# szaguldo-kamaz/FRI-ReinforcementLearning-C

Measured on AMD Instinct MI355X. Metric: rule-distance evals/sec (rules x envs), higher is better.
Workload: dtype f64; 1 GPU; cfg4_acrobot_64k_x_8k_per_gpu; nant=5, universe_len=41, rules_per_env=65536, envs_per_gpu=8192, exact_hits=4, dist_backend=none, world_size=1

## Files before the change

### fri-reinforcementlearning-c_amd/csrc/episode_kernel.h

```cpp
#pragma once

#include <type_traits>

#include "envs.h"
#include "sweeps.h"

namespace frirl {

struct NoIo {};
struct ExtIo : frirl_hip_agent_io {
    const int32_t *teacher;
};
template <bool EXT>
using IoArg = std::conditional_t<EXT, ExtIo, NoIo>;

__device__ __forceinline__ int taught_action(const ExtIo &io, int e, int A, int chosen)
{
    if (!io.teacher) return chosen;
    const int32_t k = io.teacher[e];
    return (k >= 0 && k < A) ? k : chosen;
}

struct StepShared {
    double q_ant[FRIRL_HIP_MAX_NANT];
// ... 10 lines not shown
};

__device__ __forceinline__ bool frirl_no_spread_candidates(const frirl_hip_agent &ag) { return (ag.debug_flags & 1) != 0; }

template <int NANT, int BLOCK, bool TRACK = false, class COLS, class POW>
__device__ int update_sarsa_block(const COLS &cols, const double *__restrict__ u, const double *__restrict__ ve, int U, double *__restrict__ base,
                                  int maxR, int32_t *nrules_e, const frirl_hip_agent &ag, StepShared &sh, double reward,
                                  bool qp_known, double qp, int32_t *fus_e, double *rant_e, BlockRed<BLOCK> &red,
                                  const QResult *rn_known, uint16_t *uidx_e, POW p, SpreadCand *slot, double *spread_ant_e = nullptr, int32_t *spread_R_e = nullptr)
{
    const int R = *nrules_e;
    double q1[NANT], q2[NANT];
#pragma unroll
    for (int k = 0; k < NANT; k++) { q1[k] = sh.ve1[k]; q2[k] = sh.ve2[k]; }
    double *qcol = base + (size_t)NANT * maxR;

    if (!qp_known) {
        const QResult rp = sweep_q<NANT, BLOCK>(cols, qcol, R, q2, p, red);
        qp = (rp.hit != FRIRL_HIP_NO_HIT) ? qcol[rp.hit] : rp.vagc / rp.ws;
    }
    const QResult rn = rn_known ? *rn_known : sweep_q<NANT, BLOCK, TRACK>(cols, qcol, R, q1, p, red, ag.weight_significant, slot);
    const double qnow = (rn.hit != FRIRL_HIP_NO_HIT) ? qcol[rn.hit] : rn.vagc / rn.ws;
    const double qdiff = ag.alpha * (reward + ag.gamma * qp - qnow);
    int fus = *fus_e;
    __syncthreads();

    if (qdiff > ag.qdiff_pos_boundary || qdiff < ag.qdiff_neg_boundary) {
        if (threadIdx.x < NANT) {
            const int k = threadIdx.x;
            const double r = check_possible_states(sh.q_ant[k], ag.grid_values + (size_t)k * FRIRL_HIP_MAX_GRID, ag.grid_len[k]);
            sh.rant[k] = r;
            const double *uni = u + (size_t)k * U;
            const unsigned j = snap_index(uni, U, r, universe_div(uni, U));
            sh.idx3[k] = j;
            sh.ve3[k] = ve[(size_t)k * U + j];
        }
        __syncthreads();
        double q3[NANT];
        bool same = true;
#pragma unroll
        for (int k = 0; k < NANT; k++) { q3[k] = sh.ve3[k]; same = same && (q3[k] == q1[k]); }
        QResult rr = rn;
        if (!same) rr = sweep_q<NANT, BLOCK>(cols, qcol, R, q3, p, red);
        if (rr.hit == FRIRL_HIP_NO_HIT) {
            if (R >= maxR) return FRIRL_HIP_UPD_FULL;
            const double rconc = rr.vagc / rr.ws;
            if (threadIdx.x < NANT) {
                base[(size_t)threadIdx.x * maxR + R] = q3[threadIdx.x];
                if (uidx_e) uidx_e[(size_t)threadIdx.x * maxR + R] = (uint16_t)sh.idx3[threadIdx.x];
                if (rant_e) rant_e[(size_t)threadIdx.x * maxR + R] = sh.rant[threadIdx.x];
            }
            if (threadIdx.x == 0) {
                qcol[R] = rconc + qdiff;
                *nrules_e = R + 1;
                *fus_e = 1;
            }
            return FRIRL_HIP_UPD_INSERTED;
        }
        fus = 0;
    }

    int rules = R;
    if (fus) rules--;
    int status;
    if (rn.hit != FRIRL_HIP_NO_HIT && (ag.skip_rules == 0 || (ag.skip_rules == 1 && (int)rn.hit < rules))) {
        if (threadIdx.x == 0) qcol[rn.hit] = qnow + qdiff;
        status = FRIRL_HIP_UPD_EXACT;
    } else if (ag.skip_rules == 1 && rn.hit != FRIRL_HIP_NO_HIT && (int)rn.hit == rules) {
        status = FRIRL_HIP_UPD_SKIPPED;
    } else {
        if (ag.skip_rules == 0) fus = 0;
        const int r_skip = fus ? R - 1 : -1;
        if (rn.hit == FRIRL_HIP_NO_HIT) {
            if (spread_ant_e && threadIdx.x < NANT) spread_ant_e[threadIdx.x] = sh.q_ant[threadIdx.x];
            if (spread_R_e && threadIdx.x == 0) *spread_R_e = R;
        }
        const bool from_cand = TRACK && rn.tracked && rn.hit == FRIRL_HIP_NO_HIT && !frirl_no_spread_candidates(ag) &&
                               spread_from_candidates<BLOCK>(slot[threadIdx.x], qcol, rn.ws, qnow, qdiff, ag.weight_significant, r_skip, red);
        if (!from_cand) sweep_update<NANT, BLOCK>(cols, qcol, R, q1, p, rn.ws, qnow, qdiff, ag.weight_significant, r_skip);
        status = FRIRL_HIP_UPD_SPREAD;
    }
    if (threadIdx.x == 0) *fus_e = fus;
    return status;
}

template <int NANT, int AMAX, int BLOCK, bool IDX, bool PN, bool EXT = false>
__global__ __launch_bounds__(BLOCK) void episode_begin_kernel(const double *__restrict__ u, const double *__restrict__ ve, int U,
                                                               const double *__restrict__ rb, const uint16_t *__restrict__ uidx,
                                                               const int32_t *__restrict__ nrules,
                                                               int maxR, const frirl_hip_agent ag, const frirl_hip_envs ev, const IoArg<EXT> io)
{
    constexpr int NS = NANT - 1;
    const int e = blockIdx.x;
    if constexpr (EXT) {
        if (io.reset && !io.reset[e]) return;
    }
    extern __shared__ double tab_s[];
    __shared__ double q_s[NS];
    __shared__ GbaScratch<AMAX, BLOCK> gs;
    if (IDX) for (int i = threadIdx.x; i < NANT * U; i += BLOCK) tab_s[i] = ve[i];
    if (threadIdx.x < NS) {
        double v;
        if constexpr (EXT) v = io.obs[(size_t)e * NS + threadIdx.x];
        else v = ev.start_states ? ev.start_states[(size_t)e * NS + threadIdx.x] : ag.values_def[threadIdx.x];
        ev.states[(size_t)e * NS + threadIdx.x] = v;
        ev.q_ant[(size_t)e * NANT + threadIdx.x] = v;
        q_s[threadIdx.x] = observe_ve(u, ve, U, threadIdx.x, v);
    }
    if ((int)threadIdx.x < ag.A) gs.ave[threadIdx.x] = ag.action_ve[threadIdx.x];
    __syncthreads();
    double q[NS];
#pragma unroll
    for (int k = 0; k < NS; k++) q[k] = q_s[k];
    const double *base = rb + (size_t)e * (NANT + 1) * maxR;
    const double *qcol = base + (size_t)NANT * maxR;
    const auto cols = ColsSel<IDX>::make(base, uidx + (IDX ? (size_t)e * NANT * maxR : 0), tab_s, maxR, U);
    const auto pw = PowSel<PN, NANT>::make(ag.p > 0 ? ag.p : NANT);
    int a0;
    if constexpr (AMAX == 24) {
        __shared__ BlockRed<BLOCK> red;
        double dummy[NANT] = {};
        a0 = sweep_gba_many<NANT, AMAX, BLOCK, false>(cols, qcol, nrules[e], q, dummy, pw, ag.A, gs, red, nullptr);
    } else if constexpr (AMAX > 8) {
        __shared__ BlockRed<BLOCK> red;
        double dummy[NANT] = {};
        a0 = sweep_gba_wide<NANT, 8, AMAX, BLOCK, false>(cols, qcol, nrules[e], q, dummy, pw, ag.A, gs, red, nullptr);
    } else {
        a0 = sweep_gba<NANT, AMAX, BLOCK>(cols, qcol, nrules[e], q, pw, ag.A, gs);
    }
    if (threadIdx.x == 0) {
        const uint32_t epi = ev.episode ? (uint32_t)(ev.episode[e] + 1) : 0u;
        if (ev.episode) ev.episode[e] = (int32_t)epi;
        a0 = e_greedy(ag, a0, (uint32_t)e, epi, 0u);
        if constexpr (EXT) a0 = taught_action(io, e, ag.A, a0);
        ev.q_ant[(size_t)e * NANT + NS] = ag.grid_values[(size_t)NS * FRIRL_HIP_MAX_GRID + a0];
        if constexpr (EXT) {
            io.action_out[e] = ag.grid_values[(size_t)NS * FRIRL_HIP_MAX_GRID + a0];
            if (io.action_idx) io.action_idx[e] = a0;
        }
        ev.done[e] = 0;
        ev.ep_steps[e] = 0;
        ev.ep_reward[e] = 0.0;
        if (ev.status) ev.status[e] = FRIRL_HIP_UPD_INACTIVE;
    }
}

#ifndef FRIRL_STEP_WAVES_N3
#define FRIRL_STEP_WAVES_N3 6
#endif
#ifndef FRIRL_STEP_SAME_CELL
#define FRIRL_STEP_SAME_CELL 1
#endif
constexpr int step_min_waves(int nant, int amax) { return (nant <= 3 && amax <= 4) ? FRIRL_STEP_WAVES_N3 : (amax > 8 ? 3 : 4); }

#ifdef FRIRL_STEP_TIMING
static __device__ long long g_step_timing[4 * 65536];
#endif

template <int NANT, int AMAX, int BLOCK, bool IDX, bool PN, bool TRACK, bool EXT = false>
__global__ __launch_bounds__(BLOCK, step_min_waves(NANT, AMAX)) void episode_step_kernel(const double *__restrict__ u, const double *__restrict__ ve, int U,
                                                              double *__restrict__ rb, uint16_t *__restrict__ uidx, int32_t *__restrict__ nrules,
                                                              int maxR, const frirl_hip_agent ag, const frirl_hip_envs ev, const IoArg<EXT> io)
{
    constexpr int NS = NANT - 1;
    const int e = blockIdx.x;
#ifdef FRIRL_STEP_TIMING
    static_assert(!EXT, "step timing: demo kernels only");
    const long long tm0 = wall_clock64();
#endif
    if (ev.done[e]) {
        if (threadIdx.x == 0 && ev.status) ev.status[e] = FRIRL_HIP_UPD_INACTIVE;
        return;
    }
    extern __shared__ double tab_s[];
    __shared__ StepShared sh;
    __shared__ BlockRed<BLOCK> red;
    __shared__ GbaScratch<AMAX, BLOCK> gs;
    __shared__ SpreadCand cand_s[TRACK ? BLOCK : 1];
    if (IDX) for (int i = threadIdx.x; i < NANT * U; i += BLOCK) tab_s[i] = ve[i];
    if (threadIdx.x == 0) {
        double s[FRIRL_HIP_MAX_NANT], q[FRIRL_HIP_MAX_NANT];
        if constexpr (EXT) {
            (void)s;
            for (int i = 0; i < NANT; i++) sh.q_ant[i] = ev.q_ant[(size_t)e * NANT + i];
            for (int i = 0; i < NS; i++) sh.cur_states[i] = io.obs[(size_t)e * NS + i];
            sh.reward = io.reward[e];
            sh.success = io.success[e];
            if (io.q_obs) for (int i = 0; i < NS; i++) q[i] = io.q_obs[(size_t)e * NS + i];
            else env_quantize(FRIRL_HIP_ENV_EXTERNAL, NS, ag.grid_values, ag.grid_len, ag.grid_div, sh.cur_states, q);
        } else {
            for (int i = 0; i < NS; i++) s[i] = ev.states[(size_t)e * NS + i];
            for (int i = 0; i < NANT; i++) sh.q_ant[i] = ev.q_ant[(size_t)e * NANT + i];
            env_do_action(ag.env_kind, sh.q_ant[NS], s, sh.cur_states);
            env_get_reward(ag.env_kind, sh.cur_states, sh.reward, sh.success);
            env_quantize(ag.env_kind, NS, ag.grid_values, ag.grid_len, ag.grid_div, sh.cur_states, q);
        }
        for (int i = 0; i < NS; i++) sh.cur_q_ant[i] = q[i];
    }
    if ((int)threadIdx.x < ag.A) gs.ave[threadIdx.x] = ag.action_ve[threadIdx.x];
    __syncthreads();
    if (threadIdx.x < NANT) sh.ve1[threadIdx.x] = observe_ve(u, ve, U, threadIdx.x, sh.q_ant[threadIdx.x]);
    if (threadIdx.x < NS) sh.ve2[threadIdx.x] = observe_ve(u, ve, U, threadIdx.x, sh.cur_q_ant[threadIdx.x]);
    __syncthreads();
    double q[NS];
#pragma unroll
    for (int k = 0; k < NS; k++) q[k] = sh.ve2[k];
    double *base = rb + (size_t)e * (NANT + 1) * maxR;
    const double *qcol = base + (size_t)NANT * maxR;
    uint16_t *uidx_e = uidx ? uidx + (size_t)e * NANT * maxR : nullptr;
    const auto cols = ColsSel<IDX>::make(base, uidx_e, tab_s, maxR, U);
    double q1[NANT];
#pragma unroll
    for (int k = 0; k < NANT; k++) q1[k] = sh.ve1[k];
    const auto pw = PowSel<PN, NANT>::make(ag.p > 0 ? ag.p : NANT);
    QResult rn;
    int ap;
    if constexpr (AMAX == 24) ap = sweep_gba_many<NANT, AMAX, BLOCK, true>(cols, qcol, nrules[e], q, q1, pw, ag.A, gs, red, &rn);
    else if constexpr (AMAX > 8) ap = sweep_gba_wide<NANT, 8, AMAX, BLOCK, true, TRACK>(cols, qcol, nrules[e], q, q1, pw, ag.A, gs, red, &rn, ag.weight_significant, cand_s);
    else {
        bool same_cell = NS > 0 && FRIRL_STEP_SAME_CELL != 0;
#pragma unroll
        for (int k = 0; k < NS; k++) same_cell = same_cell && (q[k] == q1[k]);
        int apend = -1;
        for (int a = ag.A - 1; a >= 0; a--) if (gs.ave[a] == q1[NS]) apend = a;
        if (same_cell && apend >= 0) ap = sweep_gba_q<NANT, AMAX, BLOCK, TRACK, true>(cols, qcol, nrules[e], q, q1, pw, ag.A, gs, red, rn, ag.weight_significant, cand_s, apend);
        else ap = sweep_gba_q<NANT, AMAX, BLOCK, TRACK, false>(cols, qcol, nrules[e], q, q1, pw, ag.A, gs, red, rn, ag.weight_significant, cand_s);
    }
#ifdef FRIRL_STEP_TIMING
    const long long tm1 = wall_clock64();
#endif
    if (threadIdx.x == 0) {
        int chosen = e_greedy(ag, ap, (uint32_t)e, ev.episode ? (uint32_t)ev.episode[e] : 0u, (uint32_t)ev.ep_steps[e] + 1u);
        if constexpr (EXT) chosen = taught_action(io, e, ag.A, chosen);
        gs.best = chosen;
        sh.cur_q_ant[NS] = ag.grid_values[(size_t)NS * FRIRL_HIP_MAX_GRID + chosen];
        sh.ve2[NS] = gs.ave[chosen];
        if constexpr (EXT) {
            io.action_out[e] = sh.cur_q_ant[NS];
            if (io.action_idx) io.action_idx[e] = chosen;
        }
    }
    __syncthreads();
    const double qp = gs.actconc[gs.best];
    double *rant_e = ev.rant ? ev.rant + (size_t)e * NANT * maxR : nullptr;
    int st = FRIRL_HIP_UPD_INACTIVE;
    if (!ag.evaluate)
        st = update_sarsa_block<NANT, BLOCK, TRACK>(cols, u, ve, U, base, maxR, nrules + e, ag, sh, sh.reward, true, qp, ev.fus + e, rant_e, red, &rn, uidx_e, pw, cand_s,
                                                    ev.spread_ant ? ev.spread_ant + (size_t)e * NANT : nullptr, ev.spread_R ? ev.spread_R + e : nullptr);
    if (threadIdx.x < NS) ev.states[(size_t)e * NS + threadIdx.x] = sh.cur_states[threadIdx.x];
    if (threadIdx.x < NANT) ev.q_ant[(size_t)e * NANT + threadIdx.x] = sh.cur_q_ant[threadIdx.x];
    if (threadIdx.x == 0) {
        const int steps = ev.ep_steps[e] + 1;
        ev.ep_steps[e] = steps;
        ev.ep_reward[e] = ev.ep_reward[e] + sh.reward;
        if (sh.success == 1 || steps >= ag.max_steps) ev.done[e] = 1;
        if (ev.status) ev.status[e] = st;
#ifdef FRIRL_STEP_TIMING
        if (e < 65536) { g_step_timing[4 * e] = tm0; g_step_timing[4 * e + 1] = tm1; g_step_timing[4 * e + 2] = wall_clock64(); g_step_timing[4 * e + 3] = st; }
#endif
    }
}

template <int N, int AMAX, int BLOCK, bool BEGIN, bool EXT>
static void launch_episode_v(const frirl_hip_tables *t, const frirl_hip_rulebases *b, const frirl_hip_agent *ag, const frirl_hip_envs *ev,
                             hipStream_t s, const IoArg<EXT> &io)
{
    const bool idx = frirl::use_uidx(t, b) && (BLOCK >= 256 || sizeof(double) * t->nant * (size_t)t->U <= 4096);
    const size_t tab = idx ? sizeof(double) * t->nant * (size_t)t->U : 0;
    const bool pn = ag->p <= 0 || ag->p == N;
    constexpr bool CAN_TRACK = (N >= 4 && AMAX <= 4);
    const int st_opt = frirl_host::opts().step_track;
    const bool track = CAN_TRACK && (st_opt == 1 || (st_opt < 0 && b->maxR > 16384 + 512));
#define EP_GO(KERNEL, DYN, ...)                                                                                                                  \
    hipLaunchKernelGGL((frirl::KERNEL<N, AMAX, BLOCK, __VA_ARGS__, EXT>), dim3(b->E), dim3(BLOCK), DYN, s, t->u, t->ve, t->U, b->rb, b->uidx, b->nrules, \
                       b->maxR, *ag, *ev, io)
    if constexpr (BEGIN) {
        if (idx) { if (pn) EP_GO(episode_begin_kernel, tab, true, true); else EP_GO(episode_begin_kernel, tab, true, false); }
        else { if (pn) EP_GO(episode_begin_kernel, 0, false, true); else EP_GO(episode_begin_kernel, 0, false, false); }
    } else {
        if constexpr (CAN_TRACK) {
            if (track) {
                if (idx) { if (pn) EP_GO(episode_step_kernel, tab, true, true, true); else EP_GO(episode_step_kernel, tab, true, false, true); }
                else { if (pn) EP_GO(episode_step_kernel, 0, false, true, true); else EP_GO(episode_step_kernel, 0, false, false, true); }
                return;
            }
        }
        if (idx) { if (pn) EP_GO(episode_step_kernel, tab, true, true, false); else EP_GO(episode_step_kernel, tab, true, false, false); }
        else { if (pn) EP_GO(episode_step_kernel, 0, false, true, false); else EP_GO(episode_step_kernel, 0, false, false, false); }
    }
#undef EP_GO
}

template <int N, bool BEGIN, bool EXT = false>
static void launch_episode(const frirl_hip_tables *t, const frirl_hip_rulebases *b, const frirl_hip_agent *ag, const frirl_hip_envs *ev,
                           hipStream_t s, const IoArg<EXT> &io = IoArg<EXT>{})
{
    bool small = b->maxR <= 2048 || (b->maxR <= 16384 && b->E >= 4096);
    const int sw = frirl_host::opts().step_wave;
    if (sw >= 0) small = sw == 1;
    if (ag->A <= 4) { if (small) launch_episode_v<N, 4, 64, BEGIN, EXT>(t, b, ag, ev, s, io); else launch_episode_v<N, 4, 256, BEGIN, EXT>(t, b, ag, ev, s, io); }
    else if (ag->A <= 8) { if (small) launch_episode_v<N, 8, 64, BEGIN, EXT>(t, b, ag, ev, s, io); else launch_episode_v<N, 8, 256, BEGIN, EXT>(t, b, ag, ev, s, io); }
    else if (ag->A <= 24 && !frirl_host::opts().no_many) launch_episode_v<N, 24, 256, BEGIN, EXT>(t, b, ag, ev, s, io);
    else launch_episode_v<N, 32, 256, BEGIN, EXT>(t, b, ag, ev, s, io);
}

}
```

### fri-reinforcementlearning-c_amd/csrc/sweeps.h

```cpp
#pragma once

#include <stdlib.h>

#include <type_traits>

#include "device_common.h"

namespace frirl {

__device__ __forceinline__ double pow_int(double b, int p)
{
    double r = b;
    for (int i = 1; i < p; i++) r = r * b;
    return r;
}

template <bool UNROLLED_POWERS = false>
__device__ __forceinline__ double inv_dist_pow(double s, int p)
{
    double y = __builtin_amdgcn_rsq(s);
    const double t = s * y;
    const double e = __fma_rn(-t, y, 1.0);
    const double c = __fma_rn(0.375, e, 0.5);
    const double ce = c * e;
// ... 128 lines not shown
    using raw_t = double2;
    __device__ __forceinline__ raw_t raw(int k, int r) const { return pair(k, r); }
    __device__ __forceinline__ raw_t raw_shared(int k, int r) const { return load_col2_shared(base + (size_t)k * maxR + r); }
    __device__ __forceinline__ double2 decode(int, const raw_t &w) const { return w; }
};

#ifndef FRIRL_BUF_LOADS
#define FRIRL_BUF_LOADS 1
#endif
static constexpr int BUFFER_RSRC_DWORD3 = 0x00020000;
__device__ __forceinline__ __amdgpu_buffer_rsrc_t raw_buffer(const void *p)
{
    return __builtin_amdgcn_make_buffer_rsrc(const_cast<void *>(p), (short)0, (int)0x7fffffff, BUFFER_RSRC_DWORD3);
}
struct QColBuf {
    __amdgpu_buffer_rsrc_t rs;
    __device__ __forceinline__ explicit QColBuf(const double *qcol) : rs(raw_buffer(qcol)) {}
    __device__ __forceinline__ double2 load2(int r) const
    {
        const auto w = __builtin_amdgcn_raw_buffer_load_b128(rs, 8 * r, 0, 2);
        double2 v;
        v.x = __longlong_as_double((long long)(((unsigned long long)w[1] << 32) | w[0]));
        v.y = __longlong_as_double((long long)(((unsigned long long)w[3] << 32) | w[2]));
        return v;
    }
};

template <int HALF>
__device__ __forceinline__ double lds_table_entry(const double *tab_k, uint32_t w)
{
#if FRIRL_DECODE_MAD
    const uint32_t base = (uint32_t)(uintptr_t)(lds_cdouble *)tab_k;
    uint32_t a;
    if constexpr (HALF == 0) asm("v_mad_u32_u16 %0, %1, 8, %2 op_sel:[0,0,0,0]" : "=v"(a) : "v"(w), "s"(base));
    else asm("v_mad_u32_u16 %0, %1, 8, %2 op_sel:[1,0,0,0]" : "=v"(a) : "v"(w), "s"(base));
    return *(lds_cdouble *)(uintptr_t)a;
#else
    return tab_k[HALF ? (w >> 16) : (w & 0xFFFFu)];
#endif
}

struct ColsIdx {
    static constexpr bool GLOBAL_Q = true;
    const uint16_t *idx;
    const double *tab;
    int maxR, U;
    __device__ __forceinline__ double2 pair(int k, int r) const
    {
        const uint32_t w = __builtin_nontemporal_load(reinterpret_cast<const uint32_t *>(idx + (size_t)k * maxR + r));
        return lds_table_pair(tab + k * U, w);
    }
    using raw_t = uint32_t;
    __device__ __forceinline__ raw_t raw(int k, int r) const
    {
#if FRIRL_BUF_LOADS
        return __builtin_amdgcn_raw_buffer_load_b32(raw_buffer(idx), 2 * r, 2 * k * maxR, 2);
#else
        return __builtin_nontemporal_load(reinterpret_cast<const uint32_t *>(idx + (size_t)k * maxR + r));
#endif
    }
    __device__ __forceinline__ raw_t raw_shared(int k, int r) const { return *reinterpret_cast<const uint32_t *>(idx + (size_t)k * maxR + r); }
    __device__ __forceinline__ double2 decode(int k, raw_t w) const { return lds_table_pair(tab + k * U, w); }
};

struct ColsLds {
    static constexpr bool GLOBAL_Q = false;
    const double *base;
    int cap;
    __device__ __forceinline__ double2 pair(int k, int r) const { return *reinterpret_cast<const double2 *>(base + (size_t)k * cap + r); }
    using raw_t = double2;
    __device__ __forceinline__ raw_t raw(int k, int r) const { return pair(k, r); }
    __device__ __forceinline__ raw_t raw_shared(int k, int r) const { return pair(k, r); }
    __device__ __forceinline__ double2 decode(int, const raw_t &w) const { return w; }
};

template <bool IDX>
struct ColsSel;
template <>
struct ColsSel<false> {
    using type = ColsF64;
    static __device__ __forceinline__ type make(const double *base, const uint16_t *, const double *, int maxR, int) { return ColsF64{base, maxR}; }
};
template <>
struct ColsSel<true> {
    using type = ColsIdx;
    static __device__ __forceinline__ type make(const double *, const uint16_t *idx, const double *tab, int maxR, int U) { return ColsIdx{idx, tab, maxR, U}; }
};

static inline bool use_uidx(const frirl_hip_tables *t, const frirl_hip_rulebases *b)
{
    return b->uidx && t->U <= 65536 && sizeof(double) * t->nant * (size_t)t->U <= 48 * 1024 && b->maxR > 2048 && !frirl_host::opts().no_uidx;
}

template <int NDIM, class COLS>
__device__ __forceinline__ void sq_dist2(const COLS &cols, int r, const double (&q)[NDIM], double &a0, double &a1)
{
    double2 v[NDIM];
#pragma unroll
    for (int k = 0; k < NDIM; k++) v[k] = cols.pair(k, r);
    double d0 = q[0] - v[0].x, d1 = q[0] - v[0].y;
    a0 = d0 * d0;
    a1 = d1 * d1;
#pragma unroll
    for (int k = 1; k < NDIM; k++) {
        d0 = q[k] - v[k].x;
        d1 = q[k] - v[k].y;
        a0 = __fma_rn(d0, d0, a0);
        a1 = __fma_rn(d1, d1, a1);
    }
}

static constexpr double SPREAD_PREFILTER_SLACK = 1.0 - 1.0 / 1048576.0;

struct SpreadCand {
    double w1, w2, w3;
    unsigned r1, r2;
    __device__ __forceinline__ void clear() { w1 = w2 = w3 = 0.0; r1 = r2 = FRIRL_HIP_NO_HIT; }
    __device__ __forceinline__ void offer(double wi, unsigned r)
    {
        if (wi > w1) { w3 = w2; w2 = w1; r2 = r1; w1 = wi; r1 = r; }
        else if (wi > w2) { w3 = w2; w2 = wi; r2 = r; }
        else if (wi > w3) w3 = wi;
    }
};

__device__ __forceinline__ double wave_uniform(double v)
{
    const unsigned long long b = (unsigned long long)__double_as_longlong(v);
    const unsigned lo = (unsigned)__builtin_amdgcn_readfirstlane((int)(unsigned)b), hi = (unsigned)__builtin_amdgcn_readfirstlane((int)(unsigned)(b >> 32));
    return __longlong_as_double((long long)(((unsigned long long)hi << 32) | lo));
}

__device__ __forceinline__ void spread_track(SpreadCand *slots, double &T, double thr, double w0, double w1, unsigned r, double run)
{
    const bool p0 = w0 > T, p1 = w1 > T;
    if (__builtin_amdgcn_ballot_w64(p0 || p1) != 0ull) {
        SpreadCand *slot = slots + threadIdx.x;
        if (p0) slot->offer(w0, r);
        if (p1) slot->offer(w1, r + 1u);
        T = wave_uniform(thr * wave_sum_f64(run));
    }
}

__device__ __forceinline__ int wave_uniform_limit(int R) { return ((R + 2 * FRIRL_WAVE - 1) / (2 * FRIRL_WAVE)) * (2 * FRIRL_WAVE); }

struct QResult {
    unsigned hit;
    double vagc;
    double ws;
    bool tracked;
};

static constexpr double NO_RULE_STATE_PART = 1.0e300;
template <class POW>
__device__ __forceinline__ void q_pair(double a0, double a1, const double2 &c, unsigned r, POW pk, unsigned &best, double &sv, double &sw, double &tw0,
                                       double &tw1)
{
    if (__builtin_amdgcn_ballot_w64(a0 == 0.0 || a1 == 0.0) != 0ull) {
        if (a0 == 0.0) best = min(best, r);
        if (a1 == 0.0) best = min(best, r + 1u);
    }
    const double w0 = shepard_w(a0, pk), w1 = shepard_w(a1, pk);
    sv = __fma_rn(w0, c.x, sv);
    sw = sw + w0;
    sv = __fma_rn(w1, c.y, sv);
    sw = sw + w1;
    tw0 = w0;
    tw1 = w1;
}

template <int NANT, int BLOCK, bool TRACK = false, class COLS, class POW>
__device__ QResult sweep_q(const COLS &cols, const double *__restrict__ qcol, int R, const double (&q)[NANT], POW p, BlockRed<BLOCK> &red, double track_thr = 0.0,
                           SpreadCand *slot = nullptr)
{
    unsigned best = FRIRL_HIP_NO_HIT;
    double sv = 0.0, sw = 0.0;
    QResult res;
    res.tracked = TRACK;
    if (TRACK) slot[threadIdx.x].clear();
    track_thr = wave_uniform(track_thr * SPREAD_PREFILTER_SLACK);
    double T = 0.0;
    const auto pk = pin_pow(p);
    const int r_lim = TRACK ? wave_uniform_limit(R) : R;
    for (int r = 2 * (int)threadIdx.x; r < r_lim; r += 2 * BLOCK) {
        double tw0 = 0.0, tw1 = 0.0;
        if (!TRACK || r < R) {
            double a0, a1;
            sq_dist2<NANT>(cols, r, q, a0, a1);
            double2 c = load_col2(qcol + r);
            if (r + 1 >= R) { a1 = NO_RULE_STATE_PART; c.y = 0.0; }
            q_pair(a0, a1, c, (unsigned)r, pk, best, sv, sw, tw0, tw1);
        }
        if (TRACK) spread_track(slot, T, track_thr, tw0, tw1, (unsigned)r, sw);
    }
    res.hit = blk_min<BLOCK>(best, red);
    res.vagc = blk_sum<BLOCK>(sv, red);
    res.ws = blk_sum<BLOCK>(sw, red);
    return res;
}

template <int NANT, int BLOCK, class COLS, class POW>
__device__ void sweep_weights(const COLS &cols, int R, const double (&q)[NANT], POW p, double ws, double *__restrict__ weights)
{
    const double iws = 1.0 / ws;
    for (int r = 2 * (int)threadIdx.x; r < R; r += 2 * BLOCK) {
        double a0, a1;
        sq_dist2<NANT>(cols, r, q, a0, a1);
        const double w0 = shepard_w(a0, p) * iws;
        const double w1 = shepard_w(a1, p) * iws;
        if (r + 1 < R) {
            double2 w; w.x = w0; w.y = w1;
            *reinterpret_cast<double2 *>(weights + r) = w;
        } else weights[r] = w0;
    }
}

template <int NANT, int BLOCK, class COLS, class POW>
__device__ void sweep_update(const COLS &cols, double *__restrict__ qcol, int R, const double (&q)[NANT], POW p, double ws, double qnow,
                             double qdiff, double threshold, int r_skip)
{
    const double iws = 1.0 / ws;
    for (int r = 2 * (int)threadIdx.x; r < R; r += 2 * BLOCK) {
        double a0, a1;
        sq_dist2<NANT>(cols, r, q, a0, a1);
        const double w0 = shepard_w(a0, p) * iws;
        const double w1 = shepard_w(a1, p) * iws;
        if (w0 > threshold && r != r_skip) { const double t = qdiff * w0; qcol[r] = qnow + t; }
        if (r + 1 < R && w1 > threshold && r + 1 != r_skip) { const double t = qdiff * w1; qcol[r + 1] = qnow + t; }
    }
}

template <int BLOCK>
__device__ bool spread_from_candidates(const SpreadCand &cd, double *__restrict__ qcol, double ws, double qnow, double qdiff, double threshold, int r_skip,
                                       BlockRed<BLOCK> &red)
{
    const double iws = 1.0 / ws;
    const unsigned ovf = (cd.w3 * iws > threshold) ? 0u : 1u;
    if (blk_min<BLOCK>(ovf, red) == 0u) return false;
    if (cd.r1 != FRIRL_HIP_NO_HIT) {
        const double w = cd.w1 * iws;
        if (w > threshold && (int)cd.r1 != r_skip) { const double t = qdiff * w; qcol[cd.r1] = qnow + t; }
    }
    if (cd.r2 != FRIRL_HIP_NO_HIT) {
        const double w = cd.w2 * iws;
        if (w > threshold && (int)cd.r2 != r_skip) { const double t = qdiff * w; qcol[cd.r2] = qnow + t; }
    }
    return true;
}

template <int AMAX, int BLOCK>
struct GbaScratch {
    static constexpr int WAVES = BLOCK / FRIRL_WAVE;
    double v[WAVES][AMAX];
    double w[WAVES][AMAX];
    unsigned hit[AMAX];
    double actconc[AMAX];
    double ave[AMAX];
    double tv[AMAX], tw[AMAX];
    int best;
};

#ifndef FRIRL_GBA_FASTPATH
#define FRIRL_GBA_FASTPATH 1
#endif
template <class POW>
__device__ __forceinline__ void concl_pair_nohit(double av, const double2 &va, double s0, double s1, const double2 &c, POW p, double &sv, double &sw)
{
    const double e0 = av - va.x, e1 = av - va.y;
    const double d0 = __fma_rn(e0, e0, s0), d1 = __fma_rn(e1, e1, s1);
    const double w0 = shepard_w(d0, p), w1 = shepard_w(d1, p);
    sv = __fma_rn(w0, c.x, sv);
    sw = sw + w0;
    sv = __fma_rn(w1, c.y, sv);
    sw = sw + w1;
}
template <class POW>
__device__ __forceinline__ void concl_pair_nohit(double av, const double2 &va, double s0, double s1, const double2 &c, POW p, double &sv, double &sw, double &w0,
                                                 double &w1)
{
    const double e0 = av - va.x, e1 = av - va.y;
    const double d0 = __fma_rn(e0, e0, s0), d1 = __fma_rn(e1, e1, s1);
    w0 = shepard_w(d0, p); w1 = shepard_w(d1, p);
    sv = __fma_rn(w0, c.x, sv);
    sw = sw + w0;
    sv = __fma_rn(w1, c.y, sv);
    sw = sw + w1;
}
__device__ __forceinline__ bool wave_no_state_hit(bool second, double s0, double s1)
{
    return FRIRL_GBA_FASTPATH && __builtin_amdgcn_ballot_w64(!second || s0 == 0.0 || s1 == 0.0) == 0ull;
}

#ifndef FRIRL_STEP_PREFETCH
#define FRIRL_STEP_PREFETCH 1
#endif
static constexpr int STEP_PREFETCH = FRIRL_STEP_PREFETCH;
__device__ __forceinline__ void note_state_hits(unsigned *hit_s, const double *ave_s, int A, double s0, double s1, const double2 &va, unsigned r)
{
    if (__builtin_amdgcn_ballot_w64(s0 == 0.0 || s1 == 0.0) != 0ull) {
        for (int a = 0; a < A; a++) {
            const double ava = ave_s[a];
            if (s0 == 0.0 && ava == va.x) atomicMin(&hit_s[a], r);
            if (s1 == 0.0 && ava == va.y) atomicMin(&hit_s[a], r + 1u);
        }
    }
}

template <int NANT, int AMAX, int BLOCK, class COLS, class POW>
__device__ int sweep_gba(const COLS &cols, const double *__restrict__ qcol, int R, const double (&qs)[NANT - 1 > 0 ? NANT - 1 : 1], POW p, int A,
                         GbaScratch<AMAX, BLOCK> &s)
{
    constexpr int NS = NANT - 1;
    double sv[AMAX], sw[AMAX], av[AMAX];
#pragma unroll
    for (int a = 0; a < AMAX; a++) { sv[a] = 0.0; sw[a] = 0.0; av[a] = wave_uniform(s.ave[a < A ? a : 0]); }
    if ((int)threadIdx.x < AMAX) s.hit[threadIdx.x] = FRIRL_HIP_NO_HIT;
    __syncthreads();
    const auto pk = pin_pow(p);
    for (int r = 2 * (int)threadIdx.x; r < R; r += 2 * BLOCK) {
        double s0 = 0.0, s1 = 0.0;
        if (NS > 0) sq_dist2<(NS > 0 ? NS : 1)>(cols, r, qs, s0, s1);
        double2 va = cols.pair(NS, r);
        double2 c = load_col2(qcol + r);
        const bool second = (r + 1 < R);
        if (!second) { s1 = NO_RULE_STATE_PART; va.y = 0.0; c.y = 0.0; }
        note_state_hits(s.hit, s.ave, A, s0, s1, va, (unsigned)r);
#pragma unroll
        for (int a = 0; a < AMAX; a++)
            if (a < A) concl_pair_nohit(av[a], va, s0, s1, c, pk, sv[a], sw[a]);
    }
    const int lane = threadIdx.x & (FRIRL_WAVE - 1), wave = threadIdx.x / FRIRL_WAVE;
    wave_sum_f64_n(sv);
    wave_sum_f64_n(sw);
#pragma unroll
    for (int a = 0; a < AMAX; a++)
        if (a < A && lane == 0) { s.v[wave][a] = sv[a]; s.w[wave][a] = sw[a]; }
    __syncthreads();
    if ((int)threadIdx.x < A) {
        const int a = threadIdx.x;
        double tv = s.v[0][a], tw = s.w[0][a];
        for (int w = 1; w < GbaScratch<AMAX, BLOCK>::WAVES; w++) { tv = tv + s.v[w][a]; tw = tw + s.w[w][a]; }
        const unsigned th = s.hit[a];
        s.actconc[a] = (th != FRIRL_HIP_NO_HIT) ? qcol[th] : tv / tw;
    }
    __syncthreads();
    if (threadIdx.x == 0) {
        int best = 0;
        for (int a = 1; a < A; a++) if (s.actconc[best] < s.actconc[a]) best = a;
        s.best = best;
    }
    __syncthreads();
    return s.best;
}

template <int NANT, int AMAX, int BLOCK, bool TRACK = false, bool SAMES = false, class COLS, class POW>
__device__ int sweep_gba_q(const COLS &cols, const double *__restrict__ qcol, int R, const double (&qs_in)[NANT - 1 > 0 ? NANT - 1 : 1],
                           const double (&q1_in)[NANT], POW p, int A, GbaScratch<AMAX, BLOCK> &s, BlockRed<BLOCK> &red, QResult &qres, double track_thr = 0.0,
                           SpreadCand *slot = nullptr, int apend = 0)
{
    constexpr int NS = NANT - 1;
    double qs[NS > 0 ? NS : 1], q1[NANT];
#pragma unroll
    for (int k = 0; k < (NS > 0 ? NS : 1); k++) qs[k] = wave_uniform(qs_in[k]);
#pragma unroll
    for (int k = 0; k < NANT; k++) q1[k] = wave_uniform(q1_in[k]);
    if (TRACK) slot[threadIdx.x].clear();
    qres.tracked = TRACK;
    track_thr = wave_uniform(track_thr * SPREAD_PREFILTER_SLACK);
    double sv[AMAX], sw[AMAX], av[AMAX];
#pragma unroll
    for (int a = 0; a < AMAX; a++) { sv[a] = 0.0; sw[a] = 0.0; av[a] = wave_uniform(s.ave[a < A ? a : 0]); }
    if ((int)threadIdx.x < AMAX) s.hit[threadIdx.x] = FRIRL_HIP_NO_HIT;
    __syncthreads();
    const auto pk = pin_pow(p);
    unsigned qbest = FRIRL_HIP_NO_HIT;
    double qv = 0.0, qw = 0.0;
    constexpr int PD = STEP_PREFETCH;
    const QColBuf qb(qcol);
    auto ldq = [&](int r) {
        if constexpr (COLS::GLOBAL_Q && FRIRL_BUF_LOADS) return qb.load2(r);
        else return load_col2(qcol + r);
    };
    typename COLS::raw_t nraw[PD][NANT];
    double2 nc[PD];
#pragma unroll
    for (int u = 0; u < PD; u++) {
        const int r0 = 2 * (int)threadIdx.x + u * 2 * BLOCK;
        nc[u] = double2{0.0, 0.0};
        if (r0 < R) {
#pragma unroll
            for (int k = 0; k < NANT; k++) nraw[u][k] = cols.raw(k, r0);
            nc[u] = ldq(r0);
        }
    }
    double T = 0.0;
    const int r_lim = TRACK ? wave_uniform_limit(R) : R;
    auto rule_pair = [&](const int r, typename COLS::raw_t (&sraw)[NANT], double2 &sc) {
        const bool live = !TRACK || r < R;
        const bool second = (r + 1 < R);
        double2 v[NANT];
        double2 c = {0.0, 0.0};
        double tw0 = 0.0, tw1 = 0.0;
        if (live) {
            c = sc;
#pragma unroll
            for (int k = 0; k < NANT; k++) v[k] = cols.decode(k, sraw[k]);
            if (r + PD * 2 * BLOCK < R) {
#pragma unroll
                for (int k = 0; k < NANT; k++) sraw[k] = cols.raw(k, r + PD * 2 * BLOCK);
                sc = ldq(r + PD * 2 * BLOCK);
            }
            if constexpr (!SAMES) {
                double d0 = q1[0] - v[0].x, d1 = q1[0] - v[0].y;
                double a0 = d0 * d0, a1 = d1 * d1;
#pragma unroll
                for (int k = 1; k < NANT; k++) {
                    d0 = q1[k] - v[k].x; d1 = q1[k] - v[k].y;
                    a0 = __fma_rn(d0, d0, a0); a1 = __fma_rn(d1, d1, a1);
                }
                if (!second) { a1 = NO_RULE_STATE_PART; c.y = 0.0; }
                q_pair(a0, a1, c, (unsigned)r, pk, qbest, qv, qw, tw0, tw1);
            }
        }
        if constexpr (!SAMES) { if (TRACK) spread_track(slot, T, track_thr, tw0, tw1, (unsigned)r, qw); }
        if (live) {
            double s0, s1;
            {
                double d0 = qs[0] - v[0].x, d1 = qs[0] - v[0].y;
                s0 = d0 * d0; s1 = d1 * d1;
#pragma unroll
                for (int k = 1; k < NS; k++) {
                    d0 = qs[k] - v[k].x; d1 = qs[k] - v[k].y;
                    s0 = __fma_rn(d0, d0, s0); s1 = __fma_rn(d1, d1, s1);
                }
            }
            double2 va = v[NS];
            if (!second) { s1 = NO_RULE_STATE_PART; va.y = 0.0; c.y = 0.0; }
            note_state_hits(s.hit, s.ave, A, s0, s1, va, (unsigned)r);
#pragma unroll
            for (int a = 0; a < AMAX; a++)
                if (a < A) {
                    if constexpr (SAMES && TRACK) {
                        double w0, w1;
                        concl_pair_nohit(av[a], va, s0, s1, c, pk, sv[a], sw[a], w0, w1);
                        if (a == apend) { tw0 = w0; tw1 = w1; qw = sw[a]; }
                    } else {
                        concl_pair_nohit(av[a], va, s0, s1, c, pk, sv[a], sw[a]);
                    }
                }
        }
        if constexpr (SAMES) { if (TRACK) spread_track(slot, T, track_thr, tw0, tw1, (unsigned)r, qw); }
    };
    for (int r = 2 * (int)threadIdx.x; r < r_lim; r += PD * 2 * BLOCK) {
#pragma unroll
        for (int u = 0; u < PD; u++) {
            const int ru = r + u * 2 * BLOCK;
            if (ru < r_lim) rule_pair(ru, nraw[u], nc[u]);
        }
    }
    if constexpr (!SAMES) {
        qres.hit = blk_min<BLOCK>(qbest, red);
        qres.vagc = blk_sum<BLOCK>(qv, red);
        qres.ws = blk_sum<BLOCK>(qw, red);
    }
    const int lane = threadIdx.x & (FRIRL_WAVE - 1), wave = threadIdx.x / FRIRL_WAVE;
    wave_sum_f64_n(sv);
    wave_sum_f64_n(sw);
#pragma unroll
    for (int a = 0; a < AMAX; a++)
        if (a < A && lane == 0) { s.v[wave][a] = sv[a]; s.w[wave][a] = sw[a]; }
    __syncthreads();
    if ((int)threadIdx.x < A) {
        const int a = threadIdx.x;
        double tv = s.v[0][a], tw = s.w[0][a];
        for (int w = 1; w < GbaScratch<AMAX, BLOCK>::WAVES; w++) { tv = tv + s.v[w][a]; tw = tw + s.w[w][a]; }
        const unsigned th = s.hit[a];
        s.actconc[a] = (th != FRIRL_HIP_NO_HIT) ? qcol[th] : tv / tw;
        s.tv[a] = tv; s.tw[a] = tw;
    }
    __syncthreads();
    if constexpr (SAMES) { qres.hit = s.hit[apend]; qres.vagc = s.tv[apend]; qres.ws = s.tw[apend]; }
    if (threadIdx.x == 0) {
        int best = 0;
        for (int a = 1; a < A; a++) if (s.actconc[best] < s.actconc[a]) best = a;
        s.best = best;
    }
    __syncthreads();
    return s.best;
}

template <int NANT, int AMAX, int BLOCK, bool WITH_Q, class COLS, class POW>
__device__ int sweep_gba_many(const COLS &cols, const double *__restrict__ qcol, int R, const double (&qs)[NANT - 1 > 0 ? NANT - 1 : 1],
                              const double (&q1)[NANT], POW p, int A, GbaScratch<AMAX, BLOCK> &s, BlockRed<BLOCK> &red, QResult *qres)
{
    constexpr int NS = NANT - 1;
    constexpr int G = 3;
    static_assert(AMAX % G == 0 && AMAX % 12 == 0, "groups of three actions, reduction passes of twelve");
    const int lane = threadIdx.x & (FRIRL_WAVE - 1), wave = __builtin_amdgcn_readfirstlane((int)(threadIdx.x / FRIRL_WAVE));
    double sv[AMAX], sw[AMAX], av[AMAX];
#pragma unroll
    for (int a = 0; a < AMAX; a++) { sv[a] = 0.0; sw[a] = 0.0; av[a] = wave_uniform(s.ave[a < A ? a : A - 1]); }
    if ((int)threadIdx.x < AMAX) s.hit[threadIdx.x] = FRIRL_HIP_NO_HIT;
    __syncthreads();
    unsigned qbest = FRIRL_HIP_NO_HIT;
    double qv = 0.0, qw = 0.0;
    const auto pk = pin_pow(p);
    const QColBuf qb(qcol);
    auto ldq = [&](int r) {
        if constexpr (COLS::GLOBAL_Q && FRIRL_BUF_LOADS) return qb.load2(r);
        else return load_col2(qcol + r);
    };
    typename COLS::raw_t nraw[NANT];
    double2 nc = {0.0, 0.0};
    {
        const int r0 = 2 * (int)threadIdx.x;
        if (r0 < R) {
#pragma unroll
            for (int k = 0; k < NANT; k++) nraw[k] = cols.raw(k, r0);
            nc = ldq(r0);
        }
    }
    for (int r = 2 * (int)threadIdx.x; r < R; r += 2 * BLOCK) {
        const bool second = (r + 1 < R);
        double2 v[NANT];
        double2 c = nc;
#pragma unroll
        for (int k = 0; k < NANT; k++) v[k] = cols.decode(k, nraw[k]);
        if (r + 2 * BLOCK < R) {
#pragma unroll
            for (int k = 0; k < NANT; k++) nraw[k] = cols.raw(k, r + 2 * BLOCK);
            nc = ldq(r + 2 * BLOCK);
        }
        if (WITH_Q) {
            double d0 = q1[0] - v[0].x, d1 = q1[0] - v[0].y;
            double a0 = d0 * d0, a1 = d1 * d1;
#pragma unroll
            for (int k = 1; k < NANT; k++) {
                d0 = q1[k] - v[k].x; d1 = q1[k] - v[k].y;
                a0 = __fma_rn(d0, d0, a0); a1 = __fma_rn(d1, d1, a1);
            }
            if (!second) { a1 = NO_RULE_STATE_PART; c.y = 0.0; }
            double tw0, tw1;
            q_pair(a0, a1, c, (unsigned)r, pk, qbest, qv, qw, tw0, tw1);
        }
        double s0, s1;
        {
            double d0 = qs[0] - v[0].x, d1 = qs[0] - v[0].y;
            s0 = d0 * d0; s1 = d1 * d1;
#pragma unroll
            for (int k = 1; k < NS; k++) {
                d0 = qs[k] - v[k].x; d1 = qs[k] - v[k].y;
                s0 = __fma_rn(d0, d0, s0); s1 = __fma_rn(d1, d1, s1);
            }
        }
        double2 va = v[NS];
        if (!second) { s1 = NO_RULE_STATE_PART; va.y = 0.0; c.y = 0.0; }
        note_state_hits(s.hit, s.ave, A, s0, s1, va, (unsigned)r);
#pragma unroll
        for (int g = 0; g < AMAX / G; g++) {
            if (G * g < A) {
#pragma unroll
                for (int j = 0; j < G; j++) concl_pair_nohit(av[G * g + j], va, s0, s1, c, pk, sv[G * g + j], sw[G * g + j]);
            }
        }
    }
    if (WITH_Q) {
        qres->hit = blk_min<BLOCK>(qbest, red);
        qres->vagc = blk_sum<BLOCK>(qv, red);
        qres->ws = blk_sum<BLOCK>(qw, red);
        qres->tracked = false;
    }
#pragma unroll
    for (int a0 = 0; a0 < AMAX; a0 += 12) {
        if (a0 < A) {
            double tv[12], tw[12];
#pragma unroll
            for (int i = 0; i < 12; i++) { tv[i] = sv[a0 + i]; tw[i] = sw[a0 + i]; }
            wave_sum_f64_n(tv);
            wave_sum_f64_n(tw);
#pragma unroll
            for (int i = 0; i < 12; i++) { sv[a0 + i] = tv[i]; sw[a0 + i] = tw[i]; }
        }
    }
#pragma unroll
    for (int a = 0; a < AMAX; a++)
        if (a < A && lane == 0) { s.v[wave][a] = sv[a]; s.w[wave][a] = sw[a]; }
    __syncthreads();
    if ((int)threadIdx.x < A) {
        const int a = threadIdx.x;
        double tv = s.v[0][a], tw = s.w[0][a];
        for (int w = 1; w < GbaScratch<AMAX, BLOCK>::WAVES; w++) { tv = tv + s.v[w][a]; tw = tw + s.w[w][a]; }
        const unsigned th = s.hit[a];
        s.actconc[a] = (th != FRIRL_HIP_NO_HIT) ? qcol[th] : tv / tw;
    }
    __syncthreads();
    if (threadIdx.x == 0) {
        int best = 0;
        for (int a = 1; a < A; a++) if (s.actconc[best] < s.actconc[a]) best = a;
        s.best = best;
    }
    __syncthreads();
    return s.best;
}

#ifndef FRIRL_WIDE_SYNC
#define FRIRL_WIDE_SYNC 8
#endif
static constexpr int WIDE_SYNC = FRIRL_WIDE_SYNC;

template <int NANT, int AG, int AMAX, int BLOCK, bool WITH_Q, bool TRACK = false, class COLS, class POW>
// ... 135 lines not shown
```

Measured before the change: 522.2 billion evals/s.

## Specialize step sweep for 3-action agents with bounds-free full-wave loop body

Adds an AMAX=3 specialization (exact action count, PN-only) for NANT 3 or 5 with p equal to NANT. The rule sweep is split into a guard-free body for fully populated wave chunks and a guarded tail. Zero-distance detection now takes the min of the high words and checks it with a wave ballot. This is meant to remove per-rule bounds checks, the dynamic action loop bound and compare overhead in the hot loop, at the cost of more template instantiations and code size. The high-word test only fires for exact zeros or denormal distances, so in rare cases it may enter the hit path unnecessarily.

```diff
diff --git a/fri-reinforcementlearning-c_amd/csrc/episode_kernel.h b/fri-reinforcementlearning-c_amd/csrc/episode_kernel.h
--- a/fri-reinforcementlearning-c_amd/csrc/episode_kernel.h
+++ b/fri-reinforcementlearning-c_amd/csrc/episode_kernel.h
@@ -186,6 +186,7 @@
 #define FRIRL_STEP_SAME_CELL 1
 #endif
 constexpr int step_min_waves(int nant, int amax) { return (nant <= 3 && amax <= 4) ? FRIRL_STEP_WAVES_N3 : (amax > 8 ? 3 : 4); }
+constexpr bool step_two_bodies(int nant, bool pn) { return (nant == 3 || nant == 5) && pn; }
 
 #ifdef FRIRL_STEP_TIMING
 static __device__ long long g_step_timing[4 * 65536];
@@ -257,8 +258,8 @@
         for (int k = 0; k < NS; k++) same_cell = same_cell && (q[k] == q1[k]);
         int apend = -1;
         for (int a = ag.A - 1; a >= 0; a--) if (gs.ave[a] == q1[NS]) apend = a;
-        if (same_cell && apend >= 0) ap = sweep_gba_q<NANT, AMAX, BLOCK, TRACK, true>(cols, qcol, nrules[e], q, q1, pw, ag.A, gs, red, rn, ag.weight_significant, cand_s, apend);
-        else ap = sweep_gba_q<NANT, AMAX, BLOCK, TRACK, false>(cols, qcol, nrules[e], q, q1, pw, ag.A, gs, red, rn, ag.weight_significant, cand_s);
+        if (same_cell && apend >= 0) ap = sweep_gba_q<NANT, AMAX, BLOCK, TRACK, true, step_two_bodies(NANT, PN)>(cols, qcol, nrules[e], q, q1, pw, ag.A, gs, red, rn, ag.weight_significant, cand_s, apend);
+        else ap = sweep_gba_q<NANT, AMAX, BLOCK, TRACK, false, step_two_bodies(NANT, PN)>(cols, qcol, nrules[e], q, q1, pw, ag.A, gs, red, rn, ag.weight_significant, cand_s);
     }
 #ifdef FRIRL_STEP_TIMING
     const long long tm1 = wall_clock64();
@@ -308,20 +309,30 @@
 #define EP_GO(KERNEL, DYN, ...)                                                                                                                  \
     hipLaunchKernelGGL((frirl::KERNEL<N, AMAX, BLOCK, __VA_ARGS__, EXT>), dim3(b->E), dim3(BLOCK), DYN, s, t->u, t->ve, t->U, b->rb, b->uidx, b->nrules, \
                        b->maxR, *ag, *ev, io)
+    constexpr bool PN_ONLY = gba_exact_actions(AMAX);
+#define EP_BEGIN(DYN, IDX_)                                                                    \
+    do {                                                                                       \
+        if (pn) EP_GO(episode_begin_kernel, DYN, IDX_, true);                                  \
+        else if constexpr (!PN_ONLY) EP_GO(episode_begin_kernel, DYN, IDX_, false);            \
+    } while (0)
+#define EP_STEP(DYN, IDX_, TRACK_)                                                             \
+    do {                                                                                       \
+        if (pn) EP_GO(episode_step_kernel, DYN, IDX_, true, TRACK_);                           \
+        else if constexpr (!PN_ONLY) EP_GO(episode_step_kernel, DYN, IDX_, false, TRACK_);     \
+    } while (0)
     if constexpr (BEGIN) {
-        if (idx) { if (pn) EP_GO(episode_begin_kernel, tab, true, true); else EP_GO(episode_begin_kernel, tab, true, false); }
-        else { if (pn) EP_GO(episode_begin_kernel, 0, false, true); else EP_GO(episode_begin_kernel, 0, false, false); }
+        if (idx) EP_BEGIN(tab, true); else EP_BEGIN(0, false);
     } else {
         if constexpr (CAN_TRACK) {
             if (track) {
-                if (idx) { if (pn) EP_GO(episode_step_kernel, tab, true, true, true); else EP_GO(episode_step_kernel, tab, true, false, true); }
-                else { if (pn) EP_GO(episode_step_kernel, 0, false, true, true); else EP_GO(episode_step_kernel, 0, false, false, true); }
+                if (idx) EP_STEP(tab, true, true); else EP_STEP(0, false, true);
                 return;
             }
         }
-        if (idx) { if (pn) EP_GO(episode_step_kernel, tab, true, true, false); else EP_GO(episode_step_kernel, tab, true, false, false); }
-        else { if (pn) EP_GO(episode_step_kernel, 0, false, true, false); else EP_GO(episode_step_kernel, 0, false, false, false); }
-    }
+        if (idx) EP_STEP(tab, true, false); else EP_STEP(0, false, false);
+    }
+#undef EP_STEP
+#undef EP_BEGIN
 #undef EP_GO
 }
 
@@ -332,6 +343,12 @@
     bool small = b->maxR <= 2048 || (b->maxR <= 16384 && b->E >= 4096);
     const int sw = frirl_host::opts().step_wave;
     if (sw >= 0) small = sw == 1;
+    if constexpr (N == 3 || N == 5) {
+        if (ag->A == 3 && (ag->p <= 0 || ag->p == N)) {
+            if (small) launch_episode_v<N, 3, 64, BEGIN, EXT>(t, b, ag, ev, s, io); else launch_episode_v<N, 3, 256, BEGIN, EXT>(t, b, ag, ev, s, io);
+            return;
+        }
+    }
     if (ag->A <= 4) { if (small) launch_episode_v<N, 4, 64, BEGIN, EXT>(t, b, ag, ev, s, io); else launch_episode_v<N, 4, 256, BEGIN, EXT>(t, b, ag, ev, s, io); }
     else if (ag->A <= 8) { if (small) launch_episode_v<N, 8, 64, BEGIN, EXT>(t, b, ag, ev, s, io); else launch_episode_v<N, 8, 256, BEGIN, EXT>(t, b, ag, ev, s, io); }
     else if (ag->A <= 24 && !frirl_host::opts().no_many) launch_episode_v<N, 24, 256, BEGIN, EXT>(t, b, ag, ev, s, io);
diff --git a/fri-reinforcementlearning-c_amd/csrc/sweeps.h b/fri-reinforcementlearning-c_amd/csrc/sweeps.h
--- a/fri-reinforcementlearning-c_amd/csrc/sweeps.h
+++ b/fri-reinforcementlearning-c_amd/csrc/sweeps.h
@@ -304,11 +304,17 @@
 };
 
 static constexpr double NO_RULE_STATE_PART = 1.0e300;
-template <class POW>
+__device__ __forceinline__ bool wave_zero_high_word(double a, double b)
+{
+    const unsigned h = min((unsigned)__double2hiint(a), (unsigned)__double2hiint(b));
+    return __builtin_amdgcn_ballot_w64(h == 0u) != 0ull;
+}
+
+template <bool HIWORD = false, class POW>
 __device__ __forceinline__ void q_pair(double a0, double a1, const double2 &c, unsigned r, POW pk, unsigned &best, double &sv, double &sw, double &tw0,
                                        double &tw1)
 {
-    if (__builtin_amdgcn_ballot_w64(a0 == 0.0 || a1 == 0.0) != 0ull) {
+    if (HIWORD ? wave_zero_high_word(a0, a1) : __builtin_amdgcn_ballot_w64(a0 == 0.0 || a1 == 0.0) != 0ull) {
         if (a0 == 0.0) best = min(best, r);
         if (a1 == 0.0) best = min(best, r + 1u);
     }
@@ -400,6 +406,8 @@
     return true;
 }
 
+constexpr bool gba_exact_actions(int amax) { return amax == 3; }
+
 template <int AMAX, int BLOCK>
 struct GbaScratch {
     static constexpr int WAVES = BLOCK / FRIRL_WAVE;
@@ -447,15 +455,20 @@
 #define FRIRL_STEP_PREFETCH 1
 #endif
 static constexpr int STEP_PREFETCH = FRIRL_STEP_PREFETCH;
+#ifndef FRIRL_STEP_TWO_BODIES
+#define FRIRL_STEP_TWO_BODIES 1
+#endif
+__device__ __forceinline__ void note_state_hits_found(unsigned *hit_s, const double *ave_s, int A, double s0, double s1, const double2 &va, unsigned r)
+{
+    for (int a = 0; a < A; a++) {
+        const double ava = ave_s[a];
+        if (s0 == 0.0 && ava == va.x) atomicMin(&hit_s[a], r);
+        if (s1 == 0.0 && ava == va.y) atomicMin(&hit_s[a], r + 1u);
+    }
+}
 __device__ __forceinline__ void note_state_hits(unsigned *hit_s, const double *ave_s, int A, double s0, double s1, const double2 &va, unsigned r)
 {
-    if (__builtin_amdgcn_ballot_w64(s0 == 0.0 || s1 == 0.0) != 0ull) {
-        for (int a = 0; a < A; a++) {
-            const double ava = ave_s[a];
-            if (s0 == 0.0 && ava == va.x) atomicMin(&hit_s[a], r);
-            if (s1 == 0.0 && ava == va.y) atomicMin(&hit_s[a], r + 1u);
-        }
-    }
+    if (__builtin_amdgcn_ballot_w64(s0 == 0.0 || s1 == 0.0) != 0ull) note_state_hits_found(hit_s, ave_s, A, s0, s1, va, r);
 }
 
 template <int NANT, int AMAX, int BLOCK, class COLS, class POW>
@@ -505,12 +518,13 @@
     return s.best;
 }
 
-template <int NANT, int AMAX, int BLOCK, bool TRACK = false, bool SAMES = false, class COLS, class POW>
+template <int NANT, int AMAX, int BLOCK, bool TRACK = false, bool SAMES = false, bool TWO = false, class COLS, class POW>
 __device__ int sweep_gba_q(const COLS &cols, const double *__restrict__ qcol, int R, const double (&qs_in)[NANT - 1 > 0 ? NANT - 1 : 1],
-                           const double (&q1_in)[NANT], POW p, int A, GbaScratch<AMAX, BLOCK> &s, BlockRed<BLOCK> &red, QResult &qres, double track_thr = 0.0,
+                           const double (&q1_in)[NANT], POW p, int A_in, GbaScratch<AMAX, BLOCK> &s, BlockRed<BLOCK> &red, QResult &qres, double track_thr = 0.0,
                            SpreadCand *slot = nullptr, int apend = 0)
 {
     constexpr int NS = NANT - 1;
+    const int A = gba_exact_actions(AMAX) ? AMAX : A_in;
     double qs[NS > 0 ? NS : 1], q1[NANT];
 #pragma unroll
     for (int k = 0; k < (NS > 0 ? NS : 1); k++) qs[k] = wave_uniform(qs_in[k]);
@@ -546,10 +560,10 @@
         }
     }
     double T = 0.0;
-    const int r_lim = TRACK ? wave_uniform_limit(R) : R;
-    auto rule_pair = [&](const int r, typename COLS::raw_t (&sraw)[NANT], double2 &sc) {
-        const bool live = !TRACK || r < R;
-        const bool second = (r + 1 < R);
+    auto rule_pair = [&](auto full_c, const int r, typename COLS::raw_t (&sraw)[NANT], double2 &sc) {
+        constexpr bool FULL = decltype(full_c)::value;
+        const bool live = FULL || !(TRACK || TWO) || r < R;
+        const bool second = FULL || (r + 1 < R);
         double2 v[NANT];
         double2 c = {0.0, 0.0};
         double tw0 = 0.0, tw1 = 0.0;
@@ -571,7 +585,7 @@
                     a0 = __fma_rn(d0, d0, a0); a1 = __fma_rn(d1, d1, a1);
                 }
                 if (!second) { a1 = NO_RULE_STATE_PART; c.y = 0.0; }
-                q_pair(a0, a1, c, (unsigned)r, pk, qbest, qv, qw, tw0, tw1);
+                q_pair<TWO>(a0, a1, c, (unsigned)r, pk, qbest, qv, qw, tw0, tw1);
             }
         }
         if constexpr (!SAMES) { if (TRACK) spread_track(slot, T, track_thr, tw0, tw1, (unsigned)r, qw); }
@@ -588,26 +602,53 @@
             }
             double2 va = v[NS];
             if (!second) { s1 = NO_RULE_STATE_PART; va.y = 0.0; c.y = 0.0; }
-            note_state_hits(s.hit, s.ave, A, s0, s1, va, (unsigned)r);
+            if constexpr (TWO) { if (wave_zero_high_word(s0, s1)) note_state_hits_found(s.hit, s.ave, A, s0, s1, va, (unsigned)r); }
+            else note_state_hits(s.hit, s.ave, A, s0, s1, va, (unsigned)r);
 #pragma unroll
             for (int a = 0; a < AMAX; a++)
                 if (a < A) {
                     if constexpr (SAMES && TRACK) {
                         double w0, w1;
                         concl_pair_nohit(av[a], va, s0, s1, c, pk, sv[a], sw[a], w0, w1);
-                        if (a == apend) { tw0 = w0; tw1 = w1; qw = sw[a]; }
+                        if (a == apend) {
+                            if constexpr (FULL) spread_track(slot, T, track_thr, w0, w1, (unsigned)r, sw[a]);
+                            else { tw0 = w0; tw1 = w1; if (!TWO) qw = sw[a]; }
+                        }
                     } else {
                         concl_pair_nohit(av[a], va, s0, s1, c, pk, sv[a], sw[a]);
                     }
                 }
         }
-        if constexpr (SAMES) { if (TRACK) spread_track(slot, T, track_thr, tw0, tw1, (unsigned)r, qw); }
+        if constexpr (SAMES && TRACK && !FULL) {
+            if constexpr (TWO) {
+#pragma unroll
+                for (int a = 0; a < AMAX; a++)
+                    if (a == apend) qw = sw[a];
+            }
+            spread_track(slot, T, track_thr, tw0, tw1, (unsigned)r, qw);
+        }
     };
-    for (int r = 2 * (int)threadIdx.x; r < r_lim; r += PD * 2 * BLOCK) {
+    if constexpr (!(TWO && FRIRL_STEP_TWO_BODIES)) {
+        const int r_lim = TRACK ? wave_uniform_limit(R) : R;
+        for (int r = 2 * (int)threadIdx.x; r < r_lim; r += PD * 2 * BLOCK) {
+#pragma unroll
+            for (int u = 0; u < PD; u++) {
+                const int ru = r + u * 2 * BLOCK;
+                if (ru < r_lim) rule_pair(std::false_type{}, ru, nraw[u], nc[u]);
+            }
+        }
+    } else {
+        int wbase = __builtin_amdgcn_readfirstlane(2 * (int)(threadIdx.x & ~(unsigned)(FRIRL_WAVE - 1)));
+        int r = 2 * (int)threadIdx.x;
+        for (; wbase + (PD - 1) * 2 * BLOCK + 2 * FRIRL_WAVE <= R; r += PD * 2 * BLOCK, wbase += PD * 2 * BLOCK) {
+#pragma unroll
+            for (int u = 0; u < PD; u++) rule_pair(std::true_type{}, r + u * 2 * BLOCK, nraw[u], nc[u]);
+        }
 #pragma unroll
         for (int u = 0; u < PD; u++) {
-            const int ru = r + u * 2 * BLOCK;
-            if (ru < r_lim) rule_pair(ru, nraw[u], nc[u]);
+            const int ru = r + u * 2 * BLOCK, wu = wbase + u * 2 * BLOCK;
+            if (PD > 1 && wu + 2 * FRIRL_WAVE <= R) rule_pair(std::true_type{}, ru, nraw[u], nc[u]);
+            else if (wu < R) rule_pair(std::false_type{}, ru, nraw[u], nc[u]);
         }
     }
     if constexpr (!SAMES) {
```

Result: no change. 522.3 billion evals/s (median of 3 runs) (+0.0%).
